# ttanida/rgrg

Measured on AMD Instinct MI355X. Metric: images/sec full 29-region report gen, 512x512 CXR, greedy max_len=128, higher is better.
Workload: dtype bf16; 1 GPU; full_model.generate() batch=32/GPU, 29 regions, greedy max_len=128, bf16 autocast: 16-bit detector, 16-bit decode GEMMs + K/V cache, hipGraph-captured decode step (BASELINE configs[2]); global_batch=32, parallelism=single GPU, weights=seeded random init (rgrg_amd.synth, profile bench), hipGraph_decode=True

## Files before the change

include/rgrg_hip.h:

```cpp
#ifndef RGRG_HIP_H_
#define RGRG_HIP_H_

#include <stdint.h>

#ifdef __cplusplus
extern "C" {
#endif

#define RGRG_OK 0
#define RGRG_EINVAL (-1)
#define RGRG_EHIP (-2)
#define RGRG_ESTATE (-3)

#define RGRG_ACT_NONE 0
#define RGRG_ACT_RELU 1
#define RGRG_ACT_GELU_NEW 2

const char* rgrg_last_error(void);
int rgrg_abi_version(void);
int rgrg_device_arch(int dev, char* buf, int buflen);

int rgrg_linear_f32(const float* A, const float* W, const float* scale, const float* shift, const float* R,
                    float* Y, int M, int N, int K, int ldy, int act, int splitk, float* ws, void* stream);
int rgrg_conv2d_nhwc_f32(const float* X, const float* W, const float* scale, const float* shift, const float* R,
// ... 133 lines not shown
                            float* lse, int S, int H, int T, int variant, uint64_t seed, uint32_t stream_id, float p, int fp16,
                            void* stream);
int rgrg_debug_attn_backward_f32(const float* qkv, const float* ukv, int ld_ukv, int kcol, const float* am, const float* d_att,
                                 const float* att, const float* lse, float* delta, float* d_qkv, float* d_ukv, uint16_t* d_qkv16,
                                 int S, int H, int T, uint64_t seed, uint32_t stream_id, float p, int fp16, float ukv_scale,
                                 void* stream);
int rgrg_debug_attn_train16(int backward, const uint16_t* qkv16, const uint16_t* ukv16, int ld_ukv, int kcol, const float* am,
                            uint16_t* att16, float* lse, const uint16_t* d_att16, uint16_t* d_qkv16, float* d_ukv, int S, int H,
                            int T, uint64_t seed, uint32_t stream_id, float p, float ukv_scale, int fp16, void* stream);
int rgrg_box_match_f32(const float* gt, const int* gt_count, int G, const float* boxes, int64_t box_image_stride,
                       const int* box_count, int B, int N, float high, float low, int allow_low_quality, int* matched,
                       int* ws_best_per_gt, void* stream);
int rgrg_balanced_sample(const int* matched, const int64_t* gt_labels, int G, const int* box_count, const float* keys,
                         uint64_t seed, int stage, int B, int n, int batch, int max_pos, uint32_t* ws_keys, uint8_t* mask,
                         int* list, int* count, void* stream);
int rgrg_rpn_loss_sampled_f32(const float* rpn_out, int ld, int anchors_per_cell, const int* matched, const float* gt, int G,
                              const float* anchors, const uint8_t* mask, const int* list, const int* count, int B, int A,
                              int batch, float* out2, void* stream);
int rgrg_roi_add_gt_f32(const float* props, const int* counts, int P, const float* gt, const int* gt_count, int G, int B,
                        float* boxes, int* box_count, void* stream);
int rgrg_roi_gather_samples_f32(const float* boxes, const int* matched, const float* gt, const int64_t* gt_labels,
                                const int* gt_count, int G, const int* list, const int* count, int B, int N, int K, float wx,
                                float wy, float ww, float wh, float* props_s, int* offsets, int64_t* labels_flat,
                                float* reg_targets, void* stream);
int rgrg_fastrcnn_loss_f32(const float* pred, int ld, int num_classes, const int64_t* labels, const float* reg_targets, int N,
                           float* out2, void* stream);

int rgrg_decoder_copy_last_logits(rgrg_decoder* d, float* dst, int S, void* stream);
int rgrg_decoder_time_step_parts(rgrg_decoder* d, int S, int nkeys, int iters, int one_range, float* ms_gemm, float* ms_attn,
                                 double* gemm_flops, double* gemm_weight_bytes, double* kv_bytes, int* gemm_launches);
int rgrg_decoder_trace_step(rgrg_decoder* d, int S, int nkeys, int iters, float* recs, int max_recs, int* n_out);
int rgrg_decoder_attention_only(rgrg_decoder* d, int S, int nkeys, int iters, void* stream);
int rgrg_decoder_row_limit(rgrg_decoder* d);
int rgrg_debug_chain(int n, int mode, int blocks, float* us_per_kernel);

#ifdef __cplusplus
}
#endif
#endif
```

rgrg_amd/_hip.py:

```python
from __future__ import annotations

import ctypes as C
import os
from typing import Optional

from . import build as _build

c_float_p = C.c_void_p
_i, _f, _p = C.c_int, C.c_float, C.c_void_p

ACT_NONE, ACT_RELU, ACT_GELU_NEW = 0, 1, 2
ABI_VERSION = 26


class RgrgHipError(RuntimeError):
    pass


class DecoderLayerWeights(C.Structure):
    _fields_ = [(n, _p) for n in ("ln1_g", "ln1_b", "ln2_g", "ln2_b", "c_attn_w", "c_attn_b", "attn_proj_w",
                                  "attn_proj_b", "c_fc_w", "c_fc_b", "mlp_proj_w", "mlp_proj_b")]


class DecoderWeights(C.Structure):
# ... 47 lines not shown
    "rgrg_bf16_to_f32": (_i, [_p, _p, C.c_int64, _i, _p]),
    "rgrg_conv2d_nhwc_bf16": (_i, [_p, _p, _p, _p, _p, _p, _i, _i, _i, _i, _i, _i, _i, _i, _i, _i, _i, _p]),
    "rgrg_linear_bf16w_f32": (_i, [_p, _p, _p, _p, _p, _i, _i, _i, _i, _i, _i, _p]),
    "rgrg_linear_bf16_f32": (_i, [_p, _p, _p, _p, _p, _p, _i, _i, _i, _i, _i, _i, _p]),
    "rgrg_debug_linear_bf16_tile": (_i, [_p, _p, _p, _p, _p, _i, _i, _i, _i, _i, _i, _i, _i, _i, _p]),
    "rgrg_debug_linear_bf16_train": (_i, [_p, _p, _p, _p, _p, _p, _p, _p, _i, _i, _i, _i, _i, _i, _i, _p]),
    "rgrg_debug_linear_bf16_argmax": (_i, [_p, _p, _p, _i, _i, _i, _p, _p, _i, _p]),
    "rgrg_debug_ln_fold16": (_i, [_p, _p, _p, _p, _p, _p, _p, _i, _i, _i, _p]),
    "rgrg_debug_linear_bf16_ln": (_i, [_p, _p, _p, _p, _p, _p, _p, _p, _p, _i, _i, _i, _i, _i, _i, _p]),
    "rgrg_debug_linear_bf16_ln_kp": (_i, [_p, _p, _p, _p, _p, _p, _p, _p, _p, _p, _i, _i, _i, _i, _i, _i, _i, _p]),
    "rgrg_debug_attn_decode": (_i, [_p, _i, _p, _p, _p, _p, _p, _i, _i, _i, _p, _p, _i, _i, _i, _i, _i, _p]),
    "rgrg_debug_linear_bf16_ln_kv": (_i, [_p, _p, _p, _p, _p, _p, _p, _p, _p, _i, _i, _i, _i, _i, _i, _p]),
    "rgrg_debug_attn_decode_qonly": (_i, [_p, _i, _p, _p, _p, _p, _p, _i, _i, _i, _i, _i, _p]),
    "rgrg_debug_attn_decode_first": (_i, [_p, _i, _p, _p, _p, _p, _p, _i, _i, _i, _p, _i, _i, _i, _p]),
    "rgrg_debug_attn_decode_kv8": (_i, [_p, _i, _p, _p, _p, _p, _p, _i, _i, _i, _p, _p, _i, _i, _p]),
    "rgrg_debug_attn_prefill": (_i, [_p, _p, _i, _i, _p, _p, _p, _p, _i, _i, _i, _i, C.c_uint64, C.c_uint32, _f, _i, _p]),
    "rgrg_debug_attn_backward_f32": (_i, [_p, _p, _i, _i, _p, _p, _p, _p, _p, _p, _p, _p, _i, _i, _i, C.c_uint64, C.c_uint32, _f,
                                          _i, _f, _p]),
    "rgrg_debug_attn_train16": (_i, [_i, _p, _p, _i, _i, _p, _p, _p, _p, _p, _p, _i, _i, _i, C.c_uint64, C.c_uint32, _f, _f, _i, _p]),
    "rgrg_decoder_copy_last_logits": (_i, [_p, _p, _i, _p]),
    "rgrg_box_match_f32": (_i, [_p, _p, _i, _p, C.c_int64, _p, _i, _i, _f, _f, _i, _p, _p, _p]),
    "rgrg_balanced_sample": (_i, [_p, _p, _i, _p, _p, C.c_uint64, _i, _i, _i, _i, _i, _p, _p, _p, _p, _p]),
    "rgrg_rpn_loss_sampled_f32": (_i, [_p, _i, _i, _p, _p, _i, _p, _p, _p, _p, _i, _i, _i, _p, _p]),
    "rgrg_roi_add_gt_f32": (_i, [_p, _p, _i, _p, _p, _i, _i, _p, _p, _p]),
    "rgrg_roi_gather_samples_f32": (_i, [_p, _p, _p, _p, _p, _i, _p, _p, _i, _i, _i, _f, _f, _f, _f, _p, _p, _p, _p, _p]),
    "rgrg_fastrcnn_loss_f32": (_i, [_p, _i, _i, _p, _p, _i, _p, _p]),
    "rgrg_decoder_trace_step": (_i, [_p, _i, _i, _i, _p, _i, C.POINTER(_i)]),
    "rgrg_decoder_attention_only": (_i, [_p, _i, _i, _i, _p]),
    "rgrg_decoder_row_limit": (_i, [_p]),
    "rgrg_decoder_set_lm_positions": (_i, [_p, _p, C.c_int64]),
    "rgrg_decoder_time_step_parts": (_i, [_p, _i, _i, _i, _i, C.POINTER(_f), C.POINTER(_f), C.POINTER(C.c_double),
                                          C.POINTER(C.c_double), C.POINTER(C.c_double), C.POINTER(_i)]),
    "rgrg_decoder_time_train_gemms": (_i, [_p, _i, _i, _i, C.POINTER(_f), C.POINTER(C.c_double), C.POINTER(_i)]),
    "rgrg_debug_chain": (_i, [_i, _i, _i, C.POINTER(_f)]),
}

_lib: Optional[C.CDLL] = None


def library_path() -> str:
    return _build.LIB_PATH


def load() -> C.CDLL:
    global _lib
    if _lib is not None:
        return _lib
    path = library_path()
    if _build.is_stale():
        try:
            _build.build_library()
        except Exception as e:
            if not os.path.exists(path):
                raise RgrgHipError(f"librgrg_hip.so is missing and could not be built: {e}") from e
    try:
        lib = C.CDLL(path)
    except OSError as e:
        raise RgrgHipError(f"cannot load {path}: {e} (the RGRG HIP path has no CPU fallback)") from e
    for name, (res, args) in SIGNATURES.items():
        fn = getattr(lib, name)
        fn.restype = res
        fn.argtypes = args
    got = lib.rgrg_abi_version()
    if got != ABI_VERSION:
        raise RgrgHipError(f"{path} has ABI version {got}, this package expects {ABI_VERSION}: rebuild it "
                           "(python -m rgrg_amd.build)")
# ... 24 lines not shown
```

rgrg_amd/csrc/decoder.hip:

```cpp
#include <math.h>
#include <stdlib.h>

#include <algorithm>
#include <type_traits>
#include <cmath>
#include <vector>

#include "decoder_internal.h"

namespace rgrg {

int skinny_max_rows() {
    static int v = -1;
    if (v < 0) { const char* e = getenv("RGRG_SKINNY_MAX_ROWS"); v = e ? atoi(e) : SKINNY_MAX_ROWS;
        if (v > SKINNY_MAX_ROWS) v = SKINNY_MAX_ROWS; if (v < 32) v = 32; }
    return v;
}

__global__ __launch_bounds__(256) void pack_weights_kernel(const float* __restrict__ W, float* __restrict__ P, int N,
                                                           int K, int NT) {
    const size_t total = (size_t)NT * (K / 8) * 64;
    for (size_t o = (size_t)blockIdx.x * blockDim.x + threadIdx.x; o < total; o += (size_t)gridDim.x * blockDim.x) {
        const int l = (int)(o & 63);
        const size_t t = o >> 6;
// ... 595 lines not shown
            u32x4 pk;
#pragma unroll
            for (int i = 0; i < 4; ++i) pk[i] = to16<F16>(acc[2 * i]) | (to16<F16>(acc[2 * i + 1]) << 16);
            *reinterpret_cast<u32x4*>(out16 + o) = pk;
        } else {
            *reinterpret_cast<f32x4*>(out + o) = f32x4{acc[0], acc[1], acc[2], acc[3]};
            *reinterpret_cast<f32x4*>(out + o + 4) = f32x4{acc[4], acc[5], acc[6], acc[7]};
        }
    }
    }
}

template <typename KV>
__global__ __launch_bounds__(256) void kv_slot0_kernel(const float* __restrict__ ukv, int ld, KV* __restrict__ kv_all,
                                                       size_t layer_stride, size_t kv_stride, int S, int H, int T,
                                                       int L, int row_mul, int f16) {
    const int D = H * 64;
    const size_t total = (size_t)L * 2 * S * D;
    for (size_t i = (size_t)blockIdx.x * blockDim.x + threadIdx.x; i < total; i += (size_t)gridDim.x * blockDim.x) {
        const int d = (int)(i % D);
        size_t r = i / D;
        const int s = (int)(r % S);
        r /= S;
        const int kv = (int)(r & 1), l = (int)(r >> 1);
        const int hd = d >> 6, e = d & 63;
        const float val = ukv[(size_t)s * ld + ((size_t)l * 2 + kv) * D + d];
        const size_t o = (size_t)l * layer_stride + (size_t)kv * kv_stride + (((size_t)s * row_mul * H + hd) * T) * 64 + e;
        if constexpr (sizeof(KV) == 1) kv_all[o] = (KV)f32_to_e4m3_bits(val);
        else if constexpr (sizeof(KV) == 2) kv_all[o] = (KV)to16_rt(val, f16);
        else kv_all[o] = val;
    }
}

constexpr int ARGMAX_U = 13;
__global__ __launch_bounds__(256) void argmax_update_kernel(const float* __restrict__ cand_val, const int* __restrict__ cand_idx,
                                                            int NT, long long* __restrict__ ids, int ld_ids,
                                                            int* __restrict__ finished, int* __restrict__ step,
                                                            int* __restrict__ done_len, int* __restrict__ sync, int S) {
    __shared__ float bv[4];
    __shared__ int bi[4];
    const int row = blockIdx.x, tid = threadIdx.x, lane = tid & 63, wave = tid >> 6;
    const int t = *step;
    const float* cv = cand_val + (size_t)row * NT;
    const int* cx = cand_idx + (size_t)row * NT;
    float v[ARGMAX_U];
    int ci[ARGMAX_U];
#pragma unroll
    for (int u = 0; u < ARGMAX_U; ++u) {
        const int i = min(tid + 256 * u, NT - 1);
        v[u] = cv[i];
        ci[u] = cx[i];
    }
    float best = -INFINITY;
    int idx = 0x7fffffff;
#pragma unroll
    for (int u = 0; u < ARGMAX_U; ++u)
        if (tid + 256 * u < NT && (v[u] > best || (v[u] == best && ci[u] < idx))) { best = v[u]; idx = ci[u]; }
    for (int i = tid + 256 * ARGMAX_U; i < NT; i += 256) {
        const float w = cv[i];
        const int wi = cx[i];
        if (w > best || (w == best && wi < idx)) { best = w; idx = wi; }
    }
    for (int o = 32; o > 0; o >>= 1) {
        const float ov = __shfl_xor(best, o, 64);
        const int oi = __shfl_xor(idx, o, 64);
        if (ov > best || (ov == best && oi < idx)) { best = ov; idx = oi; }
    }
    if (lane == 0) { bv[wave] = best; bi[wave] = idx; }
    __syncthreads();
    if (tid == 0) {
        for (int w = 1; w < 4; ++w)
            if (bv[w] > best || (bv[w] == best && bi[w] < idx)) { best = bv[w]; idx = bi[w]; }
        const StepBook bk{ids, ld_ids, finished, step, done_len, sync, S};
        record_step_token(bk, row, t, idx == 0x7fffffff ? 0 : idx);
    }
}

__global__ __launch_bounds__(256) void logits_candidates_kernel(const float* __restrict__ logits, int ld, int V, int NT,
                                                                float* __restrict__ cand_val, int* __restrict__ cand_idx) {
    const int row = blockIdx.y, lane = threadIdx.x & 63, wave = threadIdx.x >> 6;
    const float* x = logits + (size_t)row * ld;
    const int sub = lane & 7, tw = lane >> 3;
    constexpr int UN = 4;
    for (int t0 = (blockIdx.x * 4 + wave) * 8 * UN; t0 < NT; t0 += gridDim.x * 4 * 8 * UN) {
        f32x4 v[UN];
#pragma unroll
        for (int u = 0; u < UN; ++u) {
            const int nt = min(t0 + u * 8 + tw, NT - 1);
            v[u] = *reinterpret_cast<const f32x4*>(x + nt * 32 + sub * 4);
        }
#pragma unroll
        for (int u = 0; u < UN; ++u) {
            const int nt = t0 + u * 8 + tw;
            const int c0 = min(nt, NT - 1) * 32 + sub * 4;
            float bv = -INFINITY;
            int bi = c0;
#pragma unroll
            for (int e = 0; e < 4; ++e) {
                const float val = (c0 + e < V) ? v[u][e] : -INFINITY;
                if (val > bv) { bv = val; bi = c0 + e; }
            }
#define CAND_STEP(CTRL)                                                                                     \
    {                                                                                                       \
        const float ov = dpp_get<CTRL, 0xf>(bv);                                                            \
        const int oi = __builtin_amdgcn_update_dpp(0, bi, CTRL, 0xf, 0xf, false);                           \
        if (ov > bv || (ov == bv && oi < bi)) { bv = ov; bi = oi; }                                         \
    }
            CAND_STEP(0xB1) CAND_STEP(0x4E) CAND_STEP(0x141)
// ... 363 lines not shown
            a.Xf = cur; a.part = d->part;
            mode = DX_COMBINE4;
        }
        return direct_linear(d, w.c_attn, a, mode, S, count);
    }
    DirectArgs p{};
    p.Xf = d->att; p.Rf = nxt; p.Yf = nxt; p.act = RGRG_ACT_NONE;
    p.zero_acc = d->part;
    if ((rc = direct_linear(d, w.attn_proj, p, DX_PLAIN, S, count))) return rc;
    DirectArgs f{};
    f.Xf = nxt; f.Yf = d->ff; f.act = RGRG_ACT_GELU_NEW;
    if ((rc = direct_linear(d, w.c_fc, f, DX_PLAIN, S, count))) return rc;
    DirectArgs m{};
    m.Xf = d->ff; m.act = RGRG_ACT_NONE;
    return direct_linear(d, w.mlp_proj, m, DX_PLAIN, S, count);
}

static int enqueue_step_fused(rgrg_decoder* d, int S, bool count, const int* tok_override, const int* src, bool beam) {
    if (count) { d->gemm_bytes_per_step = 0; d->gemm_flops_per_step = 0.0; d->gemm_launches_per_step = 0; }
    hipStream_t st = d->stream;
    int rc;
    float* cur = d->x;
    float* nxt = d->x2;
    for (int l = 0; l < d->n_layer; ++l) {
        if ((rc = enqueue_layer_gemms(d, l, S, count, tok_override, cur, nxt, 0))) return rc;
        if ((rc = launch_attention(d, l, S, src, nullptr, 1))) return rc;
        if ((rc = enqueue_layer_gemms(d, l, S, count, tok_override, cur, nxt, 1))) return rc;
        float* tmp = cur; cur = nxt; nxt = tmp;
    }
    DirectArgs h{};
    h.Xf = cur; h.part = d->part; h.Y = d->logits; h.ldy = d->ld_logits; h.act = RGRG_ACT_NONE;
    if ((rc = direct_linear(d, d->lm_head, h, DX_COMBINE4, S, count, !beam))) return rc;
    if (beam) return RGRG_OK;
    hipLaunchKernelGGL(argmax_update_kernel, dim3(S), dim3(256), 0, st, d->cand_val, d->cand_idx, d->lm_head.NT, d->ids,
                       d->max_len, d->finished, d->step, d->done_len, d->sync, S);
    RGRG_LAUNCH_CHECK();
    return RGRG_OK;
}

static int range_bounds(int S, int want, int (&bounds)[MAX_CHAINS + 1]) {
    int nr = want < 1 ? 1 : (want > MAX_CHAINS ? MAX_CHAINS : want);
    const int tiles = (S + 63) / 64;
    for (; nr > 1; --nr) {
        int least = S;
        for (int i = 0; i <= nr; ++i) {
            bounds[i] = std::min(S, ((tiles * i + nr - 1) / nr) * 64);
            if (i) least = std::min(least, bounds[i] - bounds[i - 1]);
        }
        if (least > SKINNY_MAX_ROWS) break;
    }
    if (nr <= 1) { nr = 1; bounds[0] = 0; bounds[1] = S; }
    return nr;
}
template <class F>
static int run_row_ranges(rgrg_decoder* d, int S, int chains, F&& fn) {
    int bounds[MAX_CHAINS + 1];
    const int nr = range_bounds(S, chains < 0 ? -chains : chains, bounds);
    if (nr <= 1) return fn(0, S);
    if (chains > 0) {
        RGRG_HIP(hipEventRecord(d->ev_fork, d->stream));
        for (int i = 1; i < nr; ++i) RGRG_HIP(hipStreamWaitEvent(d->streams_x[i - 1], d->ev_fork, 0));
    }
    int rc = RGRG_OK;
    for (int i = 0; i < nr && !rc; ++i) {
        if (bounds[i + 1] <= bounds[i]) continue;
        if (chains > 0 && i > 0) std::swap(d->stream, d->streams_x[i - 1]);
        rc = fn(bounds[i], bounds[i + 1] - bounds[i]);
        if (chains > 0 && i > 0) std::swap(d->stream, d->streams_x[i - 1]);
    }
    if (chains > 0)
        for (int i = 1; i < nr; ++i) {
            RGRG_HIP(hipEventRecord(d->ev_join[i - 1], d->streams_x[i - 1]));
            RGRG_HIP(hipStreamWaitEvent(d->stream, d->ev_join[i - 1], 0));
        }
    return rc;
}
static int step_chains(const rgrg_decoder* d, int S, bool greedy, bool fold) {
    return (greedy && fold && S >= 512 && (d->chains < 0 || d->streams_x[0])) ? d->chains : 1;
}

static int trace_mark(rgrg_decoder* d, int r0, int tag) {
    if (!d->trace) return RGRG_OK;
    hipEvent_t e;
    RGRG_HIP(hipEventCreate(&e));
    RGRG_HIP(hipEventRecord(e, d->stream));
    d->trace->push_back({e, r0, tag});
    return RGRG_OK;
}

static bool step_ln_fold(const rgrg_decoder* d, int S) {
    return kv_is_bf16(d, S) && d->xn16 && d->ln_fold && d->ln_stat && d->layers[0].c_attn.wb_ln && d->D == 1024;
}
static bool step_qkv_cache(const rgrg_decoder* d, int S, bool plain) {
    const KvFormat f = kv_format(d, S);
    return d->qkv_cache && plain && step_ln_fold(d, S) && (f == KV_BF16 || f == KV_F16) && d->kp_gemms != 1 && d->kp_gemms != 3 && !d->key_mask_cur;
}
static GemmLnFold cons_kv_cache(const rgrg_decoder* d, const GemmLnFold& cons, int l, int r0) {
    GemmLnFold f = cons;
    u16* kcr = reinterpret_cast<u16*>(d->kv) + (size_t)l * d->kv_layer_stride + (size_t)r0 * d->H * d->T * 64;
    f.kv_k = kcr; f.kv_v = kcr + d->kv_kv_stride; f.kv_step = d->step; f.kv_H = d->H; f.kv_T = d->T;
    return f;
}

static int enqueue_head(rgrg_decoder* d, int S, bool count, bool beam, unsigned short* xn16) {
    hipStream_t st = d->stream;
    int rc;
    if (!beam && xn16 && lm_head_cand_path(d, S)) {
        GemmLnFold ce{};
        ce.cand_val = d->cand_val; ce.cand_idx = d->cand_idx;
        if ((rc = linear(d, d->lm_head, d->xn, nullptr, nullptr, S, d->ld_logits, RGRG_ACT_NONE, count, xn16, nullptr, &ce))) return rc;
        if ((rc = trace_mark(d, 0, 1002))) return rc;
        hipLaunchKernelGGL(argmax_update_kernel, dim3(S), dim3(256), 0, st, d->cand_val, d->cand_idx, (d->lm_head.N + 255) / 256, d->ids,
                           d->max_len, d->finished, d->step, d->done_len, d->sync, S);
        RGRG_LAUNCH_CHECK();
        return trace_mark(d, 0, 1003);
    }
    if ((rc = linear(d, d->lm_head, d->xn, nullptr, d->logits, S, d->ld_logits, RGRG_ACT_NONE, count, xn16))) return rc;
    if (beam) return RGRG_OK;
    const int cand_nt = (d->V + 31) / 32;
    hipLaunchKernelGGL(logits_candidates_kernel, dim3(4, S), dim3(256), 0, st, d->logits, d->ld_logits, d->V,
                       cand_nt, d->cand_val, d->cand_idx);
    RGRG_LAUNCH_CHECK();
    hipLaunchKernelGGL(argmax_update_kernel, dim3(S), dim3(256), 0, st, d->cand_val, d->cand_idx, cand_nt, d->ids,
                       d->max_len, d->finished, d->step, d->done_len, d->sync, S);
    RGRG_LAUNCH_CHECK();
    return RGRG_OK;
}
int enqueue_head_argmax(rgrg_decoder* d, int S) {
    return enqueue_head(d, S, false, false, (kv_is_bf16(d, S) && d->xn16) ? d->xn16 : nullptr);
}

int enqueue_step(rgrg_decoder* d, int S, bool count, const int* tok_override, const int* src, bool beam) {
    if (S <= decode_row_limit(d)) return enqueue_step_fused(d, S, count, tok_override, src, beam);
    if (count) { d->gemm_bytes_per_step = 0; d->gemm_flops_per_step = 0.0; d->gemm_launches_per_step = 0; }
    d->step_rows = S;
    const int D = d->D;
    int rc;
    unsigned short* xn16 = (kv_is_bf16(d, S) && d->xn16) ? d->xn16 : nullptr;
    unsigned short* att16 = xn16 ? d->att16 : nullptr;
    unsigned short* ff16 = xn16 ? d->ff16 : nullptr;
    const bool fold = step_ln_fold(d, S);
    const bool qc = step_qkv_cache(d, S, !tok_override && !src);
    static const float cons_tag = 0.f;
    GemmLnFold prod{}, cons{};
    prod.Yb16 = xn16; prod.stats_out = d->ln_stat;
    cons.ln_stats = d->ln_stat; cons.ln_colsum = &cons_tag;
    const GemmLnFold* pf = fold ? &prod : nullptr;
    const GemmLnFold* cf = fold ? &cons : nullptr;
    auto run_rows = [&](int r0, int rows) -> int {
        hipStream_t rs = d->stream;
        const size_t o = (size_t)r0 * D;
        float* x = d->x + o; float* xn = d->xn + o;
        unsigned short* xn16r = xn16 ? xn16 + o : nullptr;
        unsigned short* att16r = att16 ? att16 + o : nullptr;
        unsigned short* ff16r = ff16 ? ff16 + 4 * o : nullptr;
        float* statr = d->ln_stat ? d->ln_stat + (size_t)r0 * 32 : nullptr;
        GemmLnFold prod_r = prod, cons_r = cons;
        prod_r.Yb16 = xn16r; prod_r.stats_out = statr; cons_r.ln_stats = statr;
        const GemmLnFold* pfr = fold ? &prod_r : nullptr;
        const GemmLnFold* cfr = fold ? &cons_r : nullptr;
        hipLaunchKernelGGL(embed_ln_kernel, dim3(rows), dim3(256), 0, rs, d->wte, d->ids + (size_t)r0 * d->max_len, d->max_len, d->step,
                           d->layers[0].ln1_g, d->layers[0].ln1_b, x, xn, D, tok_override ? tok_override + r0 : nullptr, xn16r, d->f16(),
                           d->pos_override_cur ? d->pos_override_cur + r0 : nullptr, fold ? statr : (float*)nullptr);
        RGRG_LAUNCH_CHECK();
        int rc2;
        if ((rc2 = trace_mark(d, r0, 1000))) return rc2;
        for (int l = 0; l < d->n_layer; ++l) {
            const LayerW& w = d->layers[l];
            const float* ng = (l + 1 < d->n_layer) ? d->layers[l + 1].ln1_g : d->lnf_g;
            const float* nb = (l + 1 < d->n_layer) ? d->layers[l + 1].ln1_b : d->lnf_b;
            const GemmLnFold cons_kv = qc ? cons_kv_cache(d, cons_r, l, r0) : cons_r;
            if ((rc2 = linear(d, w.c_attn, xn, nullptr, d->qkv + 3 * o, rows, 3 * D, RGRG_ACT_NONE, count, xn16r, nullptr, qc ? &cons_kv : cfr))) return rc2;
            if ((rc2 = trace_mark(d, r0, l * 8 + 0))) return rc2;
            if ((rc2 = launch_attention(d, l, rows, src ? src + (size_t)r0 * d->T : nullptr, att16r, 0, r0, qc))) return rc2;
            if ((rc2 = trace_mark(d, r0, l * 8 + 1))) return rc2;
            if ((rc2 = linear(d, w.attn_proj, d->att + o, x, x, rows, D, RGRG_ACT_NONE, count, att16r, nullptr, pfr))) return rc2;
            if ((rc2 = trace_mark(d, r0, l * 8 + 2))) return rc2;
            if (!fold) {
                if ((rc2 = launch_ln_rows(x, w.ln2_g, w.ln2_b, xn, D, xn16r, d->f16(), rows, rs))) return rc2;
            }
            if ((rc2 = linear(d, w.c_fc, xn, nullptr, d->ff + 4 * o, rows, 4 * D, RGRG_ACT_GELU_NEW, count, xn16r, ff16r, cfr))) return rc2;
            if ((rc2 = trace_mark(d, r0, l * 8 + 3))) return rc2;
            if ((rc2 = linear(d, w.mlp_proj, d->ff + 4 * o, x, x, rows, D, RGRG_ACT_NONE, count, ff16r, nullptr, pfr))) return rc2;
            if ((rc2 = trace_mark(d, r0, l * 8 + 4))) return rc2;
            if (!fold || l + 1 == d->n_layer) {
                if ((rc2 = launch_ln_rows(x, ng, nb, xn, D, xn16r, d->f16(), rows, rs))) return rc2;
                if ((rc2 = trace_mark(d, r0, 1001))) return rc2;
            }
        }
        return RGRG_OK;
    };
    if ((rc = run_row_ranges(d, S, step_chains(d, S, !beam && !tok_override && !src, fold), run_rows))) return rc;
    return enqueue_head(d, S, count, beam, xn16);
}

int enqueue_prefill(rgrg_decoder* d, const float* feats, int S, int row_mul) {
    hipStream_t st = d->stream;
    const int D = d->D;
    hipLaunchKernelGGL(decode_reset_kernel, dim3(64), dim3(256), 0, st, d->ids, d->max_len, d->finished, d->step,
                       d->done_len, d->sync, S, d->max_len);
    RGRG_LAUNCH_CHECK();
    RGRG_HIP(hipMemcpyAsync(d->feats, feats, (size_t)S * D * sizeof(float), hipMemcpyDeviceToDevice, st));
    int rc;
    if ((rc = linear(d, d->fst0, d->feats, nullptr, d->h1, S, D, RGRG_ACT_RELU, false))) return rc;
    if ((rc = linear(d, d->fst2, d->h1, nullptr, d->img, S, D, RGRG_ACT_NONE, false))) return rc;
    if ((rc = linear(d, d->ukv, d->img, nullptr, d->ukv_out, S, d->ld_ukv, RGRG_ACT_NONE, false))) return rc;
    const KvFormat fmt = kv_format(d, S * row_mul);
    if (fmt == KV_E4M3)
        hipLaunchKernelGGL(kv_slot0_kernel<uint8_t>, dim3(1024), dim3(256), 0, st, d->ukv_out, d->ld_ukv,
                           reinterpret_cast<uint8_t*>(d->kv), d->kv_layer_stride, d->kv_kv_stride, S, d->H, d->T, d->n_layer, row_mul, 0);
    else if (fmt != KV_F32)
        hipLaunchKernelGGL(kv_slot0_kernel<u16>, dim3(1024), dim3(256), 0, st, d->ukv_out, d->ld_ukv,
                           reinterpret_cast<u16*>(d->kv), d->kv_layer_stride, d->kv_kv_stride, S, d->H, d->T, d->n_layer, row_mul, d->f16());
    else
        hipLaunchKernelGGL(kv_slot0_kernel<float>, dim3(1024), dim3(256), 0, st, d->ukv_out, d->ld_ukv, d->kv,
                           d->kv_layer_stride, d->kv_kv_stride, S, d->H, d->T, d->n_layer, row_mul, 0);
    RGRG_LAUNCH_CHECK();
    return RGRG_OK;
}

}

using namespace rgrg;

extern "C" size_t rgrg_decoder_kv_cache_bytes(int n_layer, int max_seqs, int max_len) {
    return (size_t)n_layer * 2 * (size_t)max_seqs * 16 * (size_t)(max_len + 1) * 64 * sizeof(float);
}

extern "C" int rgrg_decoder_create(const rgrg_decoder_weights* w, int max_seqs, int max_len, rgrg_decoder** out) {
    return rgrg_decoder_create_with_cache(w, max_seqs, max_len, nullptr, 0, out);
}

extern "C" int rgrg_decoder_create_with_cache(const rgrg_decoder_weights* w, int max_seqs, int max_len, void* kv_cache, size_t kv_cache_bytes,
                                              rgrg_decoder** out) {
    RGRG_CHECK_ARG(w && out && max_seqs > 0 && max_seqs < 65536 && max_len >= 2 && max_len <= 1024);
    RGRG_CHECK_ARG(w->d_model == 1024 && w->n_head == 16 && w->n_layer > 0 && w->vocab > 0 && w->layers);
    int rc = init_gemm_attrs();
    if (rc) return rc;
    if ((rc = init_skinny_attrs())) return rc;
    RGRG_HIP(hipDeviceSynchronize());
    rgrg_decoder* d = new rgrg_decoder();
    d->n_layer = w->n_layer; d->D = w->d_model; d->H = w->n_head; d->V = w->vocab;
    d->max_seqs = max_seqs; d->max_len = max_len; d->T = max_len + 1;
    d->rows = ((max_seqs + PAD_ROWS - 1) / PAD_ROWS) * PAD_ROWS;
    d->wte = w->wte; d->lnf_g = w->lnf_g; d->lnf_b = w->lnf_b;
    const int D = d->D;
#define TRY(x) do { rc = (x); if (rc) { rgrg_decoder_destroy(d); return rc; } } while (0)
    if (hipStreamCreateWithFlags(&d->stream, hipStreamNonBlocking) != hipSuccess ||
        hipEventCreateWithFlags(&d->ev_in, hipEventDisableTiming) != hipSuccess) {
        set_error("decoder: stream/event creation failed");
        delete d;
        return RGRG_EHIP;
    }
    if (const char* e = getenv("RGRG_GEMM_KP")) d->kp_gemms = atoi(e);
    if (const char* e = getenv("RGRG_W16_FUSED")) d->w16_fused = atoi(e) != 0;
    if (const char* e = getenv("RGRG_QKV_CACHE")) d->qkv_cache = atoi(e) != 0;
    if (const char* e = getenv("RGRG_DECODE_CHAINS")) {
        const int v = atoi(e);
        d->chains = (v >= -MAX_CHAINS && v <= MAX_CHAINS && v != 0 && v != -1) ? v : 1;
    }
    if (d->chains > 1) {
        bool ok = hipEventCreateWithFlags(&d->ev_fork, hipEventDisableTiming) == hipSuccess;
        for (int i = 0; ok && i < d->chains - 1; ++i)
            ok = hipStreamCreateWithFlags(&d->streams_x[i], hipStreamNonBlocking) == hipSuccess &&
                 hipEventCreateWithFlags(&d->ev_join[i], hipEventDisableTiming) == hipSuccess;
        if (!ok) {
            set_error("decoder: stream/event creation failed");
            rgrg_decoder_destroy(d);
            return RGRG_EHIP;
        }
    }
    if (hipHostMalloc((void**)&d->h_id_error, sizeof(int), 0) == hipSuccess) *d->h_id_error = 0;
    if (hipHostMalloc((void**)&d->h_done, 3 * sizeof(int), 0) != hipSuccess ||
        hipEventCreateWithFlags(&d->ev_poll[0], hipEventDisableTiming) != hipSuccess ||
        hipEventCreateWithFlags(&d->ev_poll[1], hipEventDisableTiming) != hipSuccess) {
        set_error("decoder: hipHostMalloc failed");
        delete d;
        return RGRG_EHIP;
    }
    TRY(make_lin(d, d->fst0, w->fst0_w, w->fst0_b, D, D, true));
    TRY(make_lin(d, d->fst2, w->fst2_w, w->fst2_b, D, D, true));
    TRY(make_lin(d, d->ukv, w->ukv_w, w->ukv_b, w->n_layer * 2 * D, D, true));
    TRY(make_lin(d, d->lm_head, w->wte, nullptr, w->vocab, D, true, true, w->lnf_g, w->lnf_b));
    d->layers.resize(w->n_layer);
    for (int l = 0; l < w->n_layer; ++l) {
        const rgrg_decoder_layer_weights& s = w->layers[l];
        LayerW& t = d->layers[l];
        t.ln1_g = s.ln1_g; t.ln1_b = s.ln1_b; t.ln2_g = s.ln2_g; t.ln2_b = s.ln2_b;
        TRY(make_lin(d, t.c_attn, s.c_attn_w, s.c_attn_b, 3 * D, D, true, true, s.ln1_g, s.ln1_b));
// ... 490 lines not shown
    return rc;
}

extern "C" int rgrg_decoder_trace_step(rgrg_decoder* d, int S, int nkeys, int iters, float* recs, int max_recs, int* n_out) {
    RGRG_CHECK_ARG(d && S > decode_row_limit(d) && S <= d->rows && nkeys >= 2 && nkeys <= d->T && recs && n_out && iters >= 0);
    d->logits_valid = false;
    std::vector<rgrg_decoder::TraceMark> marks;
    hipEvent_t base;
    RGRG_HIP(hipEventCreate(&base));
    int rc = RGRG_OK;
    for (int it = 0; it <= iters && !rc; ++it) {
        hipLaunchKernelGGL(set_int_kernel, dim3(1), dim3(64), 0, d->stream, d->step, nkeys - 2);
        if (it == iters) { d->trace = &marks; RGRG_HIP(hipEventRecord(base, d->stream)); }
        rc = enqueue_step(d, S, false);
    }
    d->trace = nullptr;
    (void)hipStreamSynchronize(d->stream);
    int n = 0;
    for (auto& m : marks) {
        float ms = 0.f;
        if (!rc && n < max_recs && hipEventElapsedTime(&ms, base, m.ev) == hipSuccess) {
            recs[3 * n] = (float)m.r0; recs[3 * n + 1] = (float)m.tag; recs[3 * n + 2] = ms;
            ++n;
        }
        (void)hipEventDestroy(m.ev);
    }
    (void)hipEventDestroy(base);
    hipLaunchKernelGGL(set_int_kernel, dim3(1), dim3(64), 0, d->stream, d->step, 0);
    (void)hipStreamSynchronize(d->stream);
    *n_out = n;
    return rc;
}

extern "C" int rgrg_decoder_time_step_parts(rgrg_decoder* d, int S, int nkeys, int iters, int one_range, float* ms_gemm, float* ms_attn,
                                            double* gemm_flops, double* gemm_weight_bytes, double* kv_bytes,
                                            int* gemm_launches) {
    RGRG_CHECK_ARG(d && S > 0 && S <= d->max_seqs && nkeys >= 2 && nkeys <= d->T && iters > 0 && ms_gemm && ms_attn);
    d->logits_valid = false;
    const int keep_chains = d->chains;
    if (one_range) d->chains = 1;
    struct Restore { rgrg_decoder* d; int c; ~Restore() { d->chains = c; } } restore{d, keep_chains};
    hipEvent_t e0, e1;
    RGRG_HIP(hipEventCreate(&e0));
    RGRG_HIP(hipEventCreate(&e1));
    const int D = d->D;
    const bool fused = d->lm_head.direct && S <= decode_row_limit(d);
    const bool bf = kv_is_bf16(d, S);
    d->step_rows = S;
    unsigned short* xn16 = (bf && d->xn16) ? d->xn16 : nullptr;
    unsigned short* att16 = xn16 ? d->att16 : nullptr;
    unsigned short* ff16 = xn16 ? d->ff16 : nullptr;
    const bool fold = step_ln_fold(d, S);
    const bool qc = step_qkv_cache(d, S, true);
    static const float cons_tag = 0.f;
    GemmLnFold prod{}, cons{};
    prod.Yb16 = xn16; prod.stats_out = d->ln_stat;
    cons.ln_stats = d->ln_stat; cons.ln_colsum = &cons_tag;
    const GemmLnFold* pf = fold ? &prod : nullptr;
    const GemmLnFold* cf = fold ? &cons : nullptr;
    int rc = RGRG_OK;
    float tg = 0.f, ta = 0.f;
    d->gemm_bytes_per_step = 0; d->gemm_flops_per_step = 0.0; d->gemm_launches_per_step = 0;
    if (qc) hipLaunchKernelGGL(set_int_kernel, dim3(1), dim3(64), 0, d->stream, d->step, nkeys - 2);
    for (int it = -1; it < iters && !rc; ++it) {
        const bool c = it == -1;
        if (it == 0) RGRG_HIP(hipEventRecord(e0, d->stream));
        rc = run_row_ranges(d, S, fused ? 1 : step_chains(d, S, true, fold), [&](int r0, int rows) -> int {
            const size_t o = (size_t)r0 * D;
            GemmLnFold prod_r = prod, cons_r = cons;
            prod_r.Yb16 = xn16 ? xn16 + o : nullptr;
            prod_r.stats_out = d->ln_stat ? d->ln_stat + (size_t)r0 * 32 : nullptr;
            cons_r.ln_stats = prod_r.stats_out;
            const GemmLnFold* pfr = pf ? &prod_r : nullptr;
            const GemmLnFold* cfr = cf ? &cons_r : nullptr;
            unsigned short* xn16r = xn16 ? xn16 + o : nullptr;
            unsigned short* att16r = att16 ? att16 + o : nullptr;
            unsigned short* ff16r = ff16 ? ff16 + 4 * o : nullptr;
            int rc2 = RGRG_OK;
            for (int l = 0; l < d->n_layer && !rc2; ++l) {
                const LayerW& w = d->layers[l];
                if (fused) {
                    if ((rc2 = enqueue_layer_gemms(d, l ? l : 1, S, c, nullptr, d->x, d->x2, 0))) break;
                    if ((rc2 = enqueue_layer_gemms(d, l, S, c, nullptr, d->x, d->x2, 1))) break;
                    continue;
                }
                const GemmLnFold cons_kv = qc ? cons_kv_cache(d, cons_r, l, r0) : cons_r;
                if ((rc2 = linear(d, w.c_attn, d->xn + o, nullptr, d->qkv + 3 * o, rows, 3 * D, RGRG_ACT_NONE, c, xn16r, nullptr, qc ? &cons_kv : cfr))) break;
                if ((rc2 = linear(d, w.attn_proj, d->att + o, d->x + o, d->h1 + o, rows, D, RGRG_ACT_NONE, c, att16r, nullptr, pfr))) break;
                if ((rc2 = linear(d, w.c_fc, d->xn + o, nullptr, d->ff + 4 * o, rows, 4 * D, RGRG_ACT_GELU_NEW, c, xn16r, ff16r, cfr))) break;
                if ((rc2 = linear(d, w.mlp_proj, d->ff + 4 * o, d->x + o, d->h1 + o, rows, D, RGRG_ACT_NONE, c, ff16r, nullptr, pfr))) break;
            }
            return rc2;
        });
        if (!rc && fused) {
            DirectArgs h{};
            h.Xf = d->x; h.part = d->part; h.Y = d->logits; h.ldy = d->ld_logits; h.act = RGRG_ACT_NONE;
            rc = direct_linear(d, d->lm_head, h, DX_COMBINE4, S, c, true);
        } else if (!rc) {
            if (xn16 && lm_head_cand_path(d, S)) {
                GemmLnFold ce{};
                ce.cand_val = d->cand_val; ce.cand_idx = d->cand_idx;
                rc = linear(d, d->lm_head, d->xn, nullptr, nullptr, S, d->ld_logits, RGRG_ACT_NONE, c, xn16, nullptr, &ce);
            } else {
                rc = linear(d, d->lm_head, d->xn, nullptr, d->logits, S, d->ld_logits, RGRG_ACT_NONE, c, xn16);
            }
        }
    }
    if (!rc) {
        RGRG_HIP(hipEventRecord(e1, d->stream));
        RGRG_HIP(hipEventSynchronize(e1));
        RGRG_HIP(hipEventElapsedTime(&tg, e0, e1));
        hipLaunchKernelGGL(set_int_kernel, dim3(1), dim3(64), 0, d->stream, d->step, nkeys - 2);
        for (int it = -1; it < iters && !rc; ++it) {
            if (it == 0) RGRG_HIP(hipEventRecord(e0, d->stream));
            rc = run_row_ranges(d, S, fused ? 1 : step_chains(d, S, true, fold), [&](int r0, int rows) -> int {
                int rc2 = RGRG_OK;
                for (int l = 0; l < d->n_layer && !rc2; ++l)
                    rc2 = launch_attention(d, l, rows, nullptr, att16 ? att16 + (size_t)r0 * D : nullptr, fused ? 1 : 0, r0, qc);
                return rc2;
            });
        }
        if (!rc) {
            RGRG_HIP(hipEventRecord(e1, d->stream));
            RGRG_HIP(hipEventSynchronize(e1));
            RGRG_HIP(hipEventElapsedTime(&ta, e0, e1));
        }
        hipLaunchKernelGGL(set_int_kernel, dim3(1), dim3(64), 0, d->stream, d->step, 0);
        (void)hipStreamSynchronize(d->stream);
    }
    (void)hipEventDestroy(e0);
    (void)hipEventDestroy(e1);
// ... 10 lines not shown
```

rgrg_amd/csrc/decoder_internal.h:

```cpp
#pragma once
#include <vector>

#include "internal.h"

namespace rgrg {

constexpr int MAX_CHAINS = 4;
constexpr int PAD_ROWS = 32;
constexpr int SKINNY_MAX_ROWS = 128;
constexpr int BOS_ID = 50256, EOS_ID = 50256, PAD_ID = 50256;
constexpr int BEAM_K = 32;
enum KvFormat { KV_F32 = 0, KV_BF16 = 1, KV_F16 = 2, KV_E4M3 = 3 };
constexpr int KV8_CHUNK_KEYS = 144;

struct StepBook {
    long long* ids;
    int ld_ids;
    int *finished, *step, *done_len, *sync;
    int S;
};
#ifdef __HIPCC__
__device__ __forceinline__ int record_step_token(const StepBook& bk, int row, int t, int tok, bool* was_finished = nullptr) {
    int fin = bk.finished[row];
    if (was_finished) *was_finished = fin != 0;
// ... 103 lines not shown
        bool a16 = false;
        bool h16 = false;
        size_t chunk = 0;
        bool seen_a16 = false, seen_a32 = false, seen_h16 = false, seen_h32 = false, seen_h16_a32 = false;
        bool have_wT = false;
        void* a16_scratch = nullptr;
        size_t a16_bytes = 0;
        void free() {
            float** fs[] = {&xs, &qkv, &ffpre, &ff, &dx, &dbig, &dxn, &logits, &dukv, &t1, &t2, &dimg, &dh1, &row_lse, &att, &lse, &delta};
            for (float** f : fs) { if (*f) (void)hipFree(*f); *f = nullptr; }
            if (count) (void)hipFree(count);
            count = nullptr;
            unsigned short** hs[] = {&xn16, &att16, &ff16, &ffpre16, &dx16, &dff16, &dqkv16, &dl16, &qkv16, &datt16, &ukv16};
            for (unsigned short** h : hs) { if (*h) (void)hipFree(*h); *h = nullptr; }
            rows = seqs = 0;
            chunk = 0;
        }
    } tr;
    int bf16_gemms = 0;
    int f16() const { return bf16_gemms == 2 ? 1 : 0; }
    unsigned short *xn16 = nullptr, *att16 = nullptr, *ff16 = nullptr;
    float* sk_ws = nullptr;
    unsigned* sk_cnt = nullptr;
    int sk_attn = 0, sk_mlp = 0;
    int step_rows = 0;
    float* ln_stat = nullptr;
    bool ln_fold = true;
    float* key_mask = nullptr;
    const float* key_mask_cur = nullptr;
    struct TraceMark { hipEvent_t ev; int r0; int tag; };
    std::vector<TraceMark>* trace = nullptr;
    bool w16_fused = true;
    bool qkv_cache = true;
    int kp_gemms = 2;
    int gemm_launches_per_step = 0;
    const int* pos_override_cur = nullptr;
    int* row_pos = nullptr;
    int* prompt_pad = nullptr;
    long long* prompt_pos = nullptr;
    const int* kv_first_cur = nullptr;
    int logits_stale_rows = 0;
    bool logits_valid = false;
    hipStream_t streams_x[rgrg::MAX_CHAINS - 1] = {};
    hipEvent_t ev_fork = nullptr, ev_join[rgrg::MAX_CHAINS - 1] = {};
    int kv8 = 0;
    int chains = 4;
};

namespace rgrg {

inline int pad256(int n) { return (n + 255) / 256 * 256; }

int dmalloc(rgrg_decoder* d, void** p, size_t bytes, bool zero);
int skinny_max_rows();
int linear(rgrg_decoder* d, const Lin& l, const float* X, const float* R, float* Y, int M, int ldy, int act,
           bool count, const unsigned short* X16 = nullptr, unsigned short* Y16 = nullptr, const GemmLnFold* ln = nullptr);
int launch_ln_rows(const float* x, const float* g, const float* b, float* xn, int D, unsigned short* xn16, int f16, int rows,
                   hipStream_t st);
int enqueue_step(rgrg_decoder* d, int S, bool count, const int* tok_override = nullptr, const int* src = nullptr,
                 bool beam = false);
int enqueue_prefill(rgrg_decoder* d, const float* feats, int S, int row_mul = 1);
int decode_begin(rgrg_decoder* d, void* stream);
int launch_attn_decode_kv8(const float* qkv, int ld_qkv, uint8_t* kc, uint8_t* vc, const int* step, float* out, unsigned short* out16,
                           int S, int H, int T, const int* src, int f16, int workgroups, hipStream_t st);
struct DecodePrologue { int (*fn)(rgrg_decoder*, int S, const void* arg); const void* arg; int steps_done; };
int run_decode_loop(rgrg_decoder* d, const float* feats, int S, int limit, int graph_key, int (*step)(rgrg_decoder*, int, bool),
// ... 11 lines not shown
```

Baseline: 88.66 images/sec.

## Run LM head and argmax per row range inside decode chains

Moves the lm_head candidate GEMM and the argmax/update kernel into each row-range chain of the multi-stream decode step, instead of running them once after all ranges join. The head work for one range can then overlap with the remaining layers of other ranges. The argmax kernel is also templated on loads per thread, with a 1-load variant used when there are at most 256 candidates. The trade-off is more, smaller lm_head GEMMs that each re-read the head weights.

```diff
diff --git a/include/rgrg_hip.h b/include/rgrg_hip.h
--- a/include/rgrg_hip.h
+++ b/include/rgrg_hip.h
@@ -189,6 +189,10 @@
 int rgrg_decoder_trace_step(rgrg_decoder* d, int S, int nkeys, int iters, float* recs, int max_recs, int* n_out);
 int rgrg_decoder_attention_only(rgrg_decoder* d, int S, int nkeys, int iters, void* stream);
 int rgrg_decoder_row_limit(rgrg_decoder* d);
+int rgrg_decoder_step_ranges(rgrg_decoder* d, int S, int* head_in_ranges);
+int rgrg_decoder_copy_last_candidates(rgrg_decoder* d, float* val, int* idx, int S, void* stream);
+int rgrg_debug_argmax_update(const float* cand_val, const int* cand_idx, int NT, int64_t* ids, int ld_ids, int* finished,
+                             int* step, int* done_len, int* sync, int S, int row0, int rows, int loads, void* stream);
 int rgrg_debug_chain(int n, int mode, int blocks, float* us_per_kernel);
 
 #ifdef __cplusplus
diff --git a/rgrg_amd/_hip.py b/rgrg_amd/_hip.py
--- a/rgrg_amd/_hip.py
+++ b/rgrg_amd/_hip.py
@@ -103,6 +103,9 @@
     "rgrg_decoder_time_step_parts": (_i, [_p, _i, _i, _i, _i, C.POINTER(_f), C.POINTER(_f), C.POINTER(C.c_double),
                                           C.POINTER(C.c_double), C.POINTER(C.c_double), C.POINTER(_i)]),
     "rgrg_decoder_time_train_gemms": (_i, [_p, _i, _i, _i, C.POINTER(_f), C.POINTER(C.c_double), C.POINTER(_i)]),
+    "rgrg_decoder_step_ranges": (_i, [_p, _i, C.POINTER(_i)]),
+    "rgrg_decoder_copy_last_candidates": (_i, [_p, _p, _p, _i, _p]),
+    "rgrg_debug_argmax_update": (_i, [_p, _p, _i, _p, _i, _p, _p, _p, _p, _i, _i, _i, _i, _p]),
     "rgrg_debug_chain": (_i, [_i, _i, _i, C.POINTER(_f)]),
 }
 
diff --git a/rgrg_amd/csrc/decoder.hip b/rgrg_amd/csrc/decoder.hip
--- a/rgrg_amd/csrc/decoder.hip
+++ b/rgrg_amd/csrc/decoder.hip
@@ -651,14 +651,14 @@
     }
 }
 
-constexpr int ARGMAX_U = 13;
+template <int ARGMAX_U>
 __global__ __launch_bounds__(256) void argmax_update_kernel(const float* __restrict__ cand_val, const int* __restrict__ cand_idx,
                                                             int NT, long long* __restrict__ ids, int ld_ids,
                                                             int* __restrict__ finished, int* __restrict__ step,
-                                                            int* __restrict__ done_len, int* __restrict__ sync, int S) {
+                                                            int* __restrict__ done_len, int* __restrict__ sync, int S, int row0) {
     __shared__ float bv[4];
     __shared__ int bi[4];
-    const int row = blockIdx.x, tid = threadIdx.x, lane = tid & 63, wave = tid >> 6;
+    const int row = row0 + blockIdx.x, tid = threadIdx.x, lane = tid & 63, wave = tid >> 6;
     const int t = *step;
     const float* cv = cand_val + (size_t)row * NT;
     const int* cx = cand_idx + (size_t)row * NT;
@@ -693,6 +693,17 @@
         const StepBook bk{ids, ld_ids, finished, step, done_len, sync, S};
         record_step_token(bk, row, t, idx == 0x7fffffff ? 0 : idx);
     }
+}
+static int launch_argmax_update(const float* cand_val, const int* cand_idx, int NT, long long* ids, int ld_ids, int* finished, int* step,
+                                int* done_len, int* sync, int S, int row0, int rows, hipStream_t st, int loads = 0) {
+    if (loads == 0) loads = NT <= 256 ? 1 : 13;
+    if (loads == 1)
+        hipLaunchKernelGGL(argmax_update_kernel<1>, dim3(rows), dim3(256), 0, st, cand_val, cand_idx, NT, ids, ld_ids, finished, step, done_len, sync, S, row0);
+    else if (loads == 13)
+        hipLaunchKernelGGL(argmax_update_kernel<13>, dim3(rows), dim3(256), 0, st, cand_val, cand_idx, NT, ids, ld_ids, finished, step, done_len, sync, S, row0);
+    else { set_error("arg-max: %d candidate loads per thread, the kernel is built for 1 and 13", loads); return RGRG_EINVAL; }
+    RGRG_LAUNCH_CHECK();
+    return RGRG_OK;
 }
 
 __global__ __launch_bounds__(256) void logits_candidates_kernel(const float* __restrict__ logits, int ld, int V, int NT,
@@ -1122,10 +1133,7 @@
     h.Xf = cur; h.part = d->part; h.Y = d->logits; h.ldy = d->ld_logits; h.act = RGRG_ACT_NONE;
     if ((rc = direct_linear(d, d->lm_head, h, DX_COMBINE4, S, count, !beam))) return rc;
     if (beam) return RGRG_OK;
-    hipLaunchKernelGGL(argmax_update_kernel, dim3(S), dim3(256), 0, st, d->cand_val, d->cand_idx, d->lm_head.NT, d->ids,
-                       d->max_len, d->finished, d->step, d->done_len, d->sync, S);
-    RGRG_LAUNCH_CHECK();
-    return RGRG_OK;
+    return launch_argmax_update(d->cand_val, d->cand_idx, d->lm_head.NT, d->ids, d->max_len, d->finished, d->step, d->done_len, d->sync, S, 0, S, st);
 }
 
 static int range_bounds(int S, int want, int (&bounds)[MAX_CHAINS + 1]) {
@@ -1192,6 +1200,10 @@
     return f;
 }
 
+static bool step_head_ranges(const rgrg_decoder* d, int S, int chains) {
+    return d->head_ranges && chains > 1 && kv_format(d, S) != KV_E4M3 && lm_head_cand_path(d, S);
+}
+
 static int enqueue_head(rgrg_decoder* d, int S, bool count, bool beam, unsigned short* xn16) {
     hipStream_t st = d->stream;
     int rc;
@@ -1200,9 +1212,8 @@
         ce.cand_val = d->cand_val; ce.cand_idx = d->cand_idx;
         if ((rc = linear(d, d->lm_head, d->xn, nullptr, nullptr, S, d->ld_logits, RGRG_ACT_NONE, count, xn16, nullptr, &ce))) return rc;
         if ((rc = trace_mark(d, 0, 1002))) return rc;
-        hipLaunchKernelGGL(argmax_update_kernel, dim3(S), dim3(256), 0, st, d->cand_val, d->cand_idx, (d->lm_head.N + 255) / 256, d->ids,
-                           d->max_len, d->finished, d->step, d->done_len, d->sync, S);
-        RGRG_LAUNCH_CHECK();
+        if ((rc = launch_argmax_update(d->cand_val, d->cand_idx, (d->lm_head.N + 255) / 256, d->ids, d->max_len, d->finished, d->step,
+                                       d->done_len, d->sync, S, 0, S, st))) return rc;
         return trace_mark(d, 0, 1003);
     }
     if ((rc = linear(d, d->lm_head, d->xn, nullptr, d->logits, S, d->ld_logits, RGRG_ACT_NONE, count, xn16))) return rc;
@@ -1211,10 +1222,7 @@
     hipLaunchKernelGGL(logits_candidates_kernel, dim3(4, S), dim3(256), 0, st, d->logits, d->ld_logits, d->V,
                        cand_nt, d->cand_val, d->cand_idx);
     RGRG_LAUNCH_CHECK();
-    hipLaunchKernelGGL(argmax_update_kernel, dim3(S), dim3(256), 0, st, d->cand_val, d->cand_idx, cand_nt, d->ids,
-                       d->max_len, d->finished, d->step, d->done_len, d->sync, S);
-    RGRG_LAUNCH_CHECK();
-    return RGRG_OK;
+    return launch_argmax_update(d->cand_val, d->cand_idx, cand_nt, d->ids, d->max_len, d->finished, d->step, d->done_len, d->sync, S, 0, S, st);
 }
 int enqueue_head_argmax(rgrg_decoder* d, int S) {
     return enqueue_head(d, S, false, false, (kv_is_bf16(d, S) && d->xn16) ? d->xn16 : nullptr);
@@ -1237,6 +1245,8 @@
     cons.ln_stats = d->ln_stat; cons.ln_colsum = &cons_tag;
     const GemmLnFold* pf = fold ? &prod : nullptr;
     const GemmLnFold* cf = fold ? &cons : nullptr;
+    const int chains = step_chains(d, S, !beam && !tok_override && !src, fold);
+    const bool head_r = step_head_ranges(d, S, chains);
     auto run_rows = [&](int r0, int rows) -> int {
         hipStream_t rs = d->stream;
         const size_t o = (size_t)r0 * D;
@@ -1278,10 +1288,18 @@
                 if ((rc2 = trace_mark(d, r0, 1001))) return rc2;
             }
         }
-        return RGRG_OK;
+        if (!head_r) return RGRG_OK;
+        GemmLnFold ce{};
+        const int nt = (d->lm_head.N + 255) / 256;
+        ce.cand_val = d->cand_val + (size_t)r0 * nt; ce.cand_idx = d->cand_idx + (size_t)r0 * nt;
+        if ((rc2 = linear(d, d->lm_head, xn, nullptr, nullptr, rows, d->ld_logits, RGRG_ACT_NONE, count, xn16r, nullptr, &ce))) return rc2;
+        if ((rc2 = trace_mark(d, r0, 1002))) return rc2;
+        if ((rc2 = launch_argmax_update(d->cand_val, d->cand_idx, nt, d->ids, d->max_len, d->finished, d->step, d->done_len, d->sync, S,
+                                        r0, rows, rs))) return rc2;
+        return trace_mark(d, r0, 1003);
     };
-    if ((rc = run_row_ranges(d, S, step_chains(d, S, !beam && !tok_override && !src, fold), run_rows))) return rc;
-    return enqueue_head(d, S, count, beam, xn16);
+    if ((rc = run_row_ranges(d, S, chains, run_rows))) return rc;
+    return head_r ? RGRG_OK : enqueue_head(d, S, count, beam, xn16);
 }
 
 int enqueue_prefill(rgrg_decoder* d, const float* feats, int S, int row_mul) {
@@ -1345,6 +1363,7 @@
     if (const char* e = getenv("RGRG_GEMM_KP")) d->kp_gemms = atoi(e);
     if (const char* e = getenv("RGRG_W16_FUSED")) d->w16_fused = atoi(e) != 0;
     if (const char* e = getenv("RGRG_QKV_CACHE")) d->qkv_cache = atoi(e) != 0;
+    if (const char* e = getenv("RGRG_HEAD_RANGES")) d->head_ranges = atoi(e) != 0;
     if (const char* e = getenv("RGRG_DECODE_CHAINS")) {
         const int v = atoi(e);
         d->chains = (v >= -MAX_CHAINS && v <= MAX_CHAINS && v != 0 && v != -1) ? v : 1;
@@ -1901,6 +1920,40 @@
     return rc;
 }
 
+extern "C" int rgrg_decoder_step_ranges(rgrg_decoder* d, int S, int* head_in_ranges) {
+    RGRG_CHECK_ARG(d && S > 0 && S <= d->max_seqs);
+    int nr = 1, head = 0;
+    if (S > decode_row_limit(d)) {
+        const int chains = step_chains(d, S, true, step_ln_fold(d, S));
+        int bounds[MAX_CHAINS + 1];
+        nr = range_bounds(S, chains < 0 ? -chains : chains, bounds);
+        head = nr > 1 && step_head_ranges(d, S, chains);
+    }
+    if (head_in_ranges) *head_in_ranges = head;
+    return nr;
+}
+
+extern "C" int rgrg_decoder_copy_last_candidates(rgrg_decoder* d, float* val, int* idx, int S, void* stream) {
+    RGRG_CHECK_ARG(d && val && idx && S > 0);
+    if (!d->logits_valid || d->logits_stale_rows < S) {
+        set_error("decoder: the last call left no arg-max candidates for %d rows (not a completed greedy generate on the candidates path)", S);
+        return RGRG_EINVAL;
+    }
+    const size_t n = (size_t)S * ((d->lm_head.N + 255) / 256);
+    RGRG_HIP(hipMemcpyAsync(val, d->cand_val, n * sizeof(float), hipMemcpyDeviceToDevice, as_stream(stream)));
+    RGRG_HIP(hipMemcpyAsync(idx, d->cand_idx, n * sizeof(int), hipMemcpyDeviceToDevice, as_stream(stream)));
+    RGRG_HIP(hipStreamSynchronize(as_stream(stream)));
+    return RGRG_OK;
+}
+
+extern "C" int rgrg_debug_argmax_update(const float* cand_val, const int* cand_idx, int NT, int64_t* ids, int ld_ids, int* finished,
+                                        int* step, int* done_len, int* sync, int S, int row0, int rows, int loads, void* stream) {
+    RGRG_CHECK_ARG(cand_val && cand_idx && NT > 0 && ids && ld_ids >= 2 && finished && step && done_len && sync);
+    RGRG_CHECK_ARG(S > 0 && S < 65536 && row0 >= 0 && rows > 0 && row0 + rows <= S && (loads == 0 || loads == 1 || loads == 13));
+    return launch_argmax_update(cand_val, cand_idx, NT, reinterpret_cast<long long*>(ids), ld_ids, finished, step, done_len, sync, S, row0, rows,
+                                as_stream(stream), loads);
+}
+
 extern "C" int rgrg_decoder_time_step_parts(rgrg_decoder* d, int S, int nkeys, int iters, int one_range, float* ms_gemm, float* ms_attn,
                                             double* gemm_flops, double* gemm_weight_bytes, double* kv_bytes,
                                             int* gemm_launches) {
@@ -1934,7 +1987,9 @@
     for (int it = -1; it < iters && !rc; ++it) {
         const bool c = it == -1;
         if (it == 0) RGRG_HIP(hipEventRecord(e0, d->stream));
-        rc = run_row_ranges(d, S, fused ? 1 : step_chains(d, S, true, fold), [&](int r0, int rows) -> int {
+        const int chains = fused ? 1 : step_chains(d, S, true, fold);
+        const bool head_r = !fused && step_head_ranges(d, S, chains);
+        rc = run_row_ranges(d, S, chains, [&](int r0, int rows) -> int {
             const size_t o = (size_t)r0 * D;
             GemmLnFold prod_r = prod, cons_r = cons;
             prod_r.Yb16 = xn16 ? xn16 + o : nullptr;
@@ -1959,13 +2014,19 @@
                 if ((rc2 = linear(d, w.c_fc, d->xn + o, nullptr, d->ff + 4 * o, rows, 4 * D, RGRG_ACT_GELU_NEW, c, xn16r, ff16r, cfr))) break;
                 if ((rc2 = linear(d, w.mlp_proj, d->ff + 4 * o, d->x + o, d->h1 + o, rows, D, RGRG_ACT_NONE, c, ff16r, nullptr, pfr))) break;
             }
+            if (!rc2 && head_r) {
+                GemmLnFold ce{};
+                const int nt = (d->lm_head.N + 255) / 256;
+                ce.cand_val = d->cand_val + (size_t)r0 * nt; ce.cand_idx = d->cand_idx + (size_t)r0 * nt;
+                rc2 = linear(d, d->lm_head, d->xn + o, nullptr, nullptr, rows, d->ld_logits, RGRG_ACT_NONE, c, xn16r, nullptr, &ce);
+            }
             return rc2;
         });
         if (!rc && fused) {
             DirectArgs h{};
             h.Xf = d->x; h.part = d->part; h.Y = d->logits; h.ldy = d->ld_logits; h.act = RGRG_ACT_NONE;
             rc = direct_linear(d, d->lm_head, h, DX_COMBINE4, S, c, true);
-        } else if (!rc) {
+        } else if (!rc && !head_r) {
             if (xn16 && lm_head_cand_path(d, S)) {
                 GemmLnFold ce{};
                 ce.cand_val = d->cand_val; ce.cand_idx = d->cand_idx;
diff --git a/rgrg_amd/csrc/decoder_internal.h b/rgrg_amd/csrc/decoder_internal.h
--- a/rgrg_amd/csrc/decoder_internal.h
+++ b/rgrg_amd/csrc/decoder_internal.h
@@ -159,6 +159,7 @@
     std::vector<TraceMark>* trace = nullptr;
     bool w16_fused = true;
     bool qkv_cache = true;
+    bool head_ranges = true;
     int kp_gemms = 2;
     int gemm_launches_per_step = 0;
     const int* pos_override_cur = nullptr;
```

Result: no change. 89.33 images/sec, median of 6 (+0.8%).
